# real-stanford/flingbot

Measured on AMD Instinct MI355X. Metric: sim steps/sec (64x64-particle cloth), higher is better.
Workload: dtype f32

## Files before the change

flingbot_amd/csrc/fs_fused_grid_kernel.h:

```cpp
#pragma once
#include "fs_fused_kernel.h"

#define FG_PLANE (FS_FUSED_MAX_PARTICLES * 4)
#define FG_PAD 1024
#define FG_OFF_XX FG_PAD
#define FG_OFF_X0 (FG_OFF_XX + 4 * FG_PLANE)
#define FG_OFF_CUR (FG_OFF_X0 + 3 * FG_PLANE)
#define FG_OFF_ITEMS (FG_OFF_CUR + FS_FUSED_CUR_BYTES)
#define FG_OFF_SCAN (FG_OFF_ITEMS + FS_FUSED_MAX_PARTICLES * 2)
#define FG_OFF_CSET (FG_OFF_SCAN + 64)
#define FG_OFF_CACC (FG_OFF_CSET + FS_FUSED_CSET_CAP * 2)
#define FG_OFF_CHIST (FG_OFF_CACC + FS_FUSED_CSET_CAP * 16)
#define FG_OFF_ROWL (FG_OFF_CHIST + 512)
#define FG_OFF_KZ (FG_OFF_ROWL + 1024)
#define FG_OFF_KS (FG_OFF_KZ + 1024)
#define FG_OFF_COLL (FG_OFF_KS + 1024)
#define FG_OFF_RCNT (FG_OFF_COLL + 512)
#define FG_LDS_BYTES (FG_OFF_RCNT + 512)
static_assert(FG_OFF_ROWL % 8 == 0 && (FG_OFF_KZ - FG_OFF_ROWL) % 8 == 0, "row tables are read as ds_read_b64 pairs");
static_assert((FG_OFF_COLL - FG_OFF_KS) % 256 == 0, "column tables share one address, rows as ds_read2st64_b32 offsets");
static_assert(FG_LDS_BYTES <= 160 * 1024, "grid-64 kernel: the LDS of one CU");
#ifndef FG_SINGLES
#define FG_SINGLES 1
#endif
#define FG_SINGLES_LANES (FS_FUSED_THREADS - 64)
#define FG_SINGLES_ROOM ((FS_FUSED_CUR_BYTES + FS_FUSED_MAX_PARTICLES * 2) / 16)
#define FG_SINGLES_CAP (FG_SINGLES_ROOM < 2 * FG_SINGLES_LANES ? FG_SINGLES_ROOM : 2 * FG_SINGLES_LANES)
#ifndef FG_PREFETCH_CAND
#define FG_PREFETCH_CAND 2
#endif

#define FG_ROW(w, k) (2 * (w) + 32 * ((k) >> 1) + ((k) & 1))

template <int DZ>
__device__ __forceinline__ void fg_load_slot(unsigned a, fs_f2 &x0, fs_f2 &x1, fs_f2 &x2) {
    asm volatile("ds_read2st64_b32 %0, %1 offset0:%2 offset1:%3" : "=v"(x0) : "v"(a), "n"(DZ + 2), "n"(DZ + 3) : "memory");
    asm volatile("ds_read2st64_b32 %0, %1 offset0:%2 offset1:%3" : "=v"(x1) : "v"(a), "n"(DZ + 2 + 64), "n"(DZ + 3 + 64) : "memory");
    asm volatile("ds_read2st64_b32 %0, %1 offset0:%2 offset1:%3" : "=v"(x2) : "v"(a), "n"(DZ + 2 + 128), "n"(DZ + 3 + 128) : "memory");
}
template <int OFF>
__device__ __forceinline__ fs_f2 fg_load_rows(unsigned a) {
    static_assert(OFF >= 0 && OFF < 65536 && OFF % 8 == 0, "ds_read_b64 offset");
    fs_f2 r;
    asm volatile("ds_read_b64 %0, %1 offset:%2" : "=v"(r) : "v"(a), "n"(OFF) : "memory");
    return r;
}
template <int R0, int R1>
__device__ __forceinline__ fs_f2 fg_load_cols(unsigned a) {
    static_assert(R0 >= 0 && R0 < 256 && R1 >= 0 && R1 < 256, "ds_read2st64_b32 offsets");
    fs_f2 r;
    asm volatile("ds_read2st64_b32 %0, %1 offset0:%2 offset1:%3" : "=v"(r) : "v"(a), "n"(R0), "n"(R1) : "memory");
    return r;
}
#define FG_WAIT(N, A0, A1, A2) asm volatile("s_waitcnt lgkmcnt(" #N ")" : "+v"(A0), "+v"(A1), "+v"(A2))

#define FG_MIN_L2 1.17549435e-38f
__device__ __forceinline__ float fg_scale(float xi0, float xi1, float xi2, float xj0, float xj1, float xj2, float L, float k,
                                          float &l2) {
    const float ex = xi0 - xj0, ey = xi1 - xj1, ez = xi2 - xj2;
    l2 = fs_dot3(ex, ey, ez, ex, ey, ez);
    const float inv = __builtin_amdgcn_rsqf(l2);
    const float len = l2 * inv;
    const float C = len - L;
    return k * (C * inv);
}
__device__ __forceinline__ void fg_accum(float &d0, float &d1, float &d2, float xi0, float xi1, float xi2, float xj0, float xj1,
                                         float xj2, float sc) {
    const float ex = xi0 - xj0, ey = xi1 - xj1, ez = xi2 - xj2;
    d0 = FS_FMA(-ex, sc, d0);
    d1 = FS_FMA(-ey, sc, d1);
    d2 = FS_FMA(-ez, sc, d2);
}
__device__ __forceinline__ float fg_from_left(float v) {
    return __int_as_float(__builtin_amdgcn_update_dpp(0, __float_as_int(v), 0x138, 0xf, 0xf, true));
}
__device__ __forceinline__ float fg_from_right(float v) {
    return __int_as_float(__builtin_amdgcn_update_dpp(0, __float_as_int(v), 0x130, 0xf, 0xf, true));
}

__device__ __forceinline__ void fg_apply(const FsAcc &a, float relax, const float *rcnt, float &x0, float &x1, float &x2) {
    if (a.cnt > 0) {
        const float sc = a.cnt < 128 ? rcnt[a.cnt] : relax / (float)a.cnt;
        x0 = FS_FMA(a.d0, sc, x0); x1 = FS_FMA(a.d1, sc, x1); x2 = FS_FMA(a.d2, sc, x2);
    }
}

__global__ __launch_bounds__(FS_FUSED_THREADS) void fs_k_fused_grid64(const FsEnvDev *__restrict__ envs,
                                                                      const FsShapesDev *__restrict__ shapes, const int *ids,
                                                                      int n_steps) {
    static_assert(FS_FUSED_THREADS == 1024 && FS_FUSED_PPT == 4, "grid-64 kernel: 16 waves x 4 rows");
    extern __shared__ __attribute__((aligned(16))) char smem[];
    float *Xx = (float *)(smem + FG_OFF_XX);
    float *Xy = Xx + FS_FUSED_MAX_PARTICLES, *Xz = Xy + FS_FUSED_MAX_PARTICLES, *Xw = Xz + FS_FUSED_MAX_PARTICLES;
    float *X0x = (float *)(smem + FG_OFF_X0);
    float *X0y = X0x + FS_FUSED_MAX_PARTICLES;
    float *X0z = X0y + FS_FUSED_MAX_PARTICLES;
    unsigned short *cursor = (unsigned short *)(smem + FG_OFF_CUR);
    unsigned short *items = (unsigned short *)(smem + FG_OFF_ITEMS);
    int *wave_tot = (int *)(smem + FG_OFF_SCAN);
    float *rowL = (float *)(smem + FG_OFF_ROWL);

#ifdef FS_BLOCK_CLOCKS
    const unsigned long long tc_start = __builtin_amdgcn_s_memtime(), tr_start = __builtin_amdgcn_s_memrealtime();
#endif
#ifdef FS_TIMING
    unsigned long long ts_acc[16] = {0, 0, 0, 0, 0, 0, 0, 0, 0, 0, 0, 0, 0, 0, 0, 0};
    unsigned long long ts_last = __builtin_amdgcn_s_memtime();
#endif
    const int e = ids[blockIdx.x];
    if (e < 0) return;
    const FsEnvDev &E = envs[e];
    const FsShapesDev &sh = shapes[e];
    const FsFusedConsts c = fs_fused_consts(E, sh);
    const int n = c.n;
    const unsigned un = (unsigned)n;
    const int t = threadIdx.x, lane = t & 63, w = t >> 6;
    const int dimz = n >> 6;

    FsVec4 *const g_pos = E.pos, *const g_vel = E.vel;
    const FsVec4 *const g_rest = E.rest;
    const fs_gci g_phase = (fs_gci)E.phase;
    const fs_gi g_nlist = (fs_gi)E.nlist, g_ncount = (fs_gi)E.ncount;
    const fs_gci g_ell_j = (fs_gci)E.ell_j;
    const fs_gcf g_ell_len = (fs_gcf)E.ell_len, g_ell_k = (fs_gcf)E.ell_k;
    const fs_gcf g_L = (fs_gcf)E.g64_L;
    const int max_deg = E.max_deg;
    const fs_gcu g_near = (fs_gcu)E.restnear_w;

    int find_mode = 0;
    {
        const int ph0 = g_phase[0];
        int differs = 0;
        for (int i = t; i < n; i += FS_FUSED_THREADS) differs |= (g_phase[i] != ph0);
        if (t == 0) wave_tot[0] = 0;
        __syncthreads();
        if (differs) atomicOr(&wave_tot[0], 1);
        __syncthreads();
        const int mixed = wave_tot[0];
        __syncthreads();
        if (!mixed) {
            if (!(ph0 & FS_PHASE_SELF_COLLIDE)) find_mode = 3;
            else if (!(ph0 & FS_PHASE_SELF_COLLIDE_FILTER)) find_mode = 2;
            else if (E.restnear_ok == 2 && FS_STENCIL_FILTER) find_mode = 4;
            else if (E.restnear_ok) find_mode = 1;
        }
    }
    for (int q = t; q < FG_OFF_X0 / 4; q += FS_FUSED_THREADS) ((float *)smem)[q] = 0.0f;
    __syncthreads();
    for (int i = t; i < n; i += FS_FUSED_THREADS) {
        const FsVec4 p = fs_ld4(g_pos, i);
        Xx[i] = p.x; Xy[i] = p.y; Xz[i] = p.z; Xw[i] = p.w;
        X0x[i] = p.x; X0y[i] = p.y; X0z[i] = p.z;
    }
    if (t < 256) {
        const int r = t & 63, s = 8 + (t >> 6);
        rowL[t] = r < dimz ? g_L[(unsigned)s * un + (unsigned)(r * 64 + 2)] : 0.0f;
    }
    constexpr int XS_DX[4] = {-1, -2, +1, +2};
    constexpr int SH_DX[4] = {+1, -1, -1, +1}, SH_DZ[4] = {-1, -1, +1, +1};
    constexpr int ZS_DZ[4] = {-1, -2, +1, +2};
    float *colL = (float *)(smem + FG_OFF_COLL);
    if (t < 128) {
        const int col = t & 63, q = t >> 6;
        const int dxq = q == 0 ? -1 : -2;
        colL[t] = (unsigned)(col + dxq) < 64u ? g_L[(unsigned)q * un + (unsigned)(2 * 64 + col)] : 0.0f;
    }
    float *rcnt = (float *)(smem + FG_OFF_RCNT);
    if (t < 128) rcnt[t] = t > 0 ? c.relax / (float)t : 0.0f;
    if (t < 256) {
        const int c64 = t & 63, q = t >> 6;
        const int sdx = (q == 0 || q == 3) ? +1 : -1, sslot = q < 2 ? 2 + q : 4 + q;
        const int zdz = q < 2 ? -1 - q : q - 1;
        ((float *)(smem + FG_OFF_KS))[t] = (unsigned)(c64 + sdx) < 64u ? E.g64_kh[sslot] : 0.0f;
        ((float *)(smem + FG_OFF_KZ))[t] = (c64 < dimz && (unsigned)(c64 + zdz) < (unsigned)dimz) ? E.g64_kh[8 + q] : 0.0f;
    }
    const float kh0 = E.g64_kh[0], kh1 = E.g64_kh[1];
    unsigned nvalid = 0u;
#pragma unroll
    for (int k = 0; k < FS_FUSED_PPT; ++k) {
        const int row = FG_ROW(w, k);
        int cnt = 0;
#pragma unroll
        for (int q = 0; q < 4; ++q) {
            cnt += ((unsigned)(lane + XS_DX[q]) < 64u) ? 1 : 0;
            cnt += ((unsigned)(lane + SH_DX[q]) < 64u && (unsigned)(row + SH_DZ[q]) < (unsigned)dimz) ? 1 : 0;
            cnt += ((unsigned)(row + ZS_DZ[q]) < (unsigned)dimz) ? 1 : 0;
        }
        nvalid |= (unsigned)cnt << (8 * k);
    }
    __syncthreads();
    unsigned fastmask = 0u;
    {
        constexpr int cdx[FS_G64_SLOTS] = FS_G64_DX_LIST, cdz[FS_G64_SLOTS] = FS_G64_DZ_LIST;
#pragma unroll
        for (int k = 0; k < FS_FUSED_PPT; ++k) {
            const int row = FG_ROW(w, k), i = row * 64 + lane;
            bool differs = false;
            if (i < n) {
                const float wi = Xw[i];
                differs = !(wi > 0.0f);
#pragma unroll
                for (int q = 0; q < FS_G64_SLOTS; ++q) {
                    const bool in = (unsigned)(lane + cdx[q]) < 64u && (unsigned)(row + cdz[q]) < (unsigned)dimz;
                    if (in) differs |= Xw[i + cdz[q] * 64 + cdx[q]] != wi;
                }
            }
            if (i < n && __builtin_amdgcn_ballot_w64(differs) == 0ull) fastmask |= 1u << k;
        }
        fastmask = (unsigned)__builtin_amdgcn_readfirstlane((int)fastmask);
    }

    FS_TS(0)
#pragma unroll 1
    for (int frame = 0; frame < n_steps; ++frame) {
#pragma unroll 1
        for (int sub = 0; sub < c.substeps; ++sub) {
            for (int q = t; q < FS_FUSED_BUCKETS / 2; q += FS_FUSED_THREADS) ((unsigned *)cursor)[q] = 0u;
            FsVec4 xp[FS_FUSED_PPT];
#pragma unroll
            for (int k = 0; k < FS_FUSED_PPT; ++k) {
                const int i = t + k * FS_FUSED_THREADS;
                xp[k] = FsVec4{0.0f, 0.0f, 0.0f, 0.0f};
                if (i < n) {
                    const FsVec4 p0 = FsVec4{X0x[i], X0y[i], X0z[i], Xw[i]};
                    xp[k] = fs_fused_predict(c, p0, fs_ld4(g_vel, i));
                    fs_st4(E.x0, i, p0);
                }
            }
            __syncthreads();
            fs_fused_build_grid(c, xp, cursor, items, wave_tot, X0x, X0y, X0z);
            FS_TS(1)
            const FsFindConsts fc = {n, c.ncap, c.rad2, c.inv_rad, find_mode, E.gp_dimx, E.gp_magic};
#pragma unroll 1
            for (int qs = t; qs < n; qs += FS_FUSED_THREADS) {
                const int i = items[qs];
                const FsVec4 xi = FsVec4{X0x[qs], X0y[qs], X0z[qs], 0.0f};
                const int shape_bits = (int)(fs_shape_candidates(E.p, sh, sub, xi.x, xi.y, xi.z) << FS_SHAPE_MASK_SHIFT);
                if (find_mode == 4) {
                    FsNearWords none;
#pragma unroll
                    for (int q = 0; q < 8; ++q) none.w[q] = 0xffffffffu;
                    g_ncount[i] = fs_fused_find_neighbors<true>(fc, i, xi, (fs_lcus)cursor, (fs_lcus)items, g_phase, g_rest, g_nlist,
                                                                none, (fs_lus)(smem + FG_OFF_XX) + t, (fs_lcf)X0x) | shape_bits;
                    continue;
                }
                FsNearWords near;
#pragma unroll
                for (int q = 0; q < 8; ++q) near.w[q] = find_mode == 1 ? g_near[(unsigned)q * un + (unsigned)i] : 0xffffffffu;
                g_ncount[i] = (find_mode == 3 ? 0
                                              : fs_fused_find_neighbors<false>(fc, i, xi, (fs_lcus)cursor, (fs_lcus)items, g_phase,
                                                                               g_rest, g_nlist, near,
                                                                               (fs_lus)(smem + FG_OFF_XX) + t, (fs_lcf)X0x)) |
                              shape_bits;
            }
            FS_TS(2)
            __syncthreads();
            FS_TS(3)
#pragma unroll
            for (int k = 0; k < FS_FUSED_PPT; ++k) {
                const int i = t + k * FS_FUSED_THREADS;
                if (i < n) {
                    Xx[i] = xp[k].x; Xy[i] = xp[k].y; Xz[i] = xp[k].z; Xw[i] = xp[k].w;
                    const FsVec4 p0 = fs_ld4(E.x0, i);
                    X0x[i] = p0.x; X0y[i] = p0.y; X0z[i] = p0.z;
                } else {
                    Xx[i] = 0.0f; Xy[i] = 0.0f; Xz[i] = 0.0f; Xw[i] = 0.0f;
                }
            }

            unsigned short *cset = (unsigned short *)(smem + FG_OFF_CSET);
            FsVec4 *cacc = (FsVec4 *)(smem + FG_OFF_CACC);
            int *chist = (int *)(smem + FG_OFF_CHIST);
            if (t < 128) chist[t] = 0;
            int *nsingles = (int *)(smem + FG_OFF_SCAN);
            if (t == 0) *nsingles = 0;
            __syncthreads();
            int ccls[FS_FUSED_PPT];
#pragma unroll
            for (int k = 0; k < FS_FUSED_PPT; ++k) {
                const int i = FG_ROW(w, k) * 64 + lane;
                int cc = 0;
                if (i < n && Xw[i] > 0.0f) cc = g_ncount[i] & FS_NCOUNT_MASK;
                ccls[k] = cc > 96 ? 96 : cc;
                if (ccls[k] > 0) atomicAdd(&chist[ccls[k]], 1);
            }
            __syncthreads();
            fs_fused_count_offsets(chist, t);
            __syncthreads();
            unsigned long long slotpack = ~0ull;
#pragma unroll
            for (int k = 0; k < FS_FUSED_PPT; ++k) {
                if (ccls[k] > 0) {
                    const int pos = atomicAdd(&chist[ccls[k]], 1);
                    if (pos < FS_FUSED_CSET_CAP) {
                        cset[pos] = (unsigned short)(FG_ROW(w, k) * 64 + lane);
                        slotpack = (slotpack & ~(0xffffull << (16 * k))) | ((unsigned long long)pos << (16 * k));
                    }
#if FG_SINGLES
                    else if (ccls[k] <= 16) {
                        const int sp = atomicAdd(nsingles, 1);
                        if (sp < FG_SINGLES_CAP)
                            slotpack = (slotpack & ~(0xffffull << (16 * k))) | ((unsigned long long)(FS_FUSED_CSET_CAP + sp) << (16 * k));
                    }
#endif
                }
            }
            __syncthreads();
            const int csize = chist[0] < FS_FUSED_CSET_CAP ? chist[0] : FS_FUSED_CSET_CAP;
            const int n_singles = *nsingles < FG_SINGLES_CAP ? *nsingles : FG_SINGLES_CAP;
            FsVec4 *squeue = (FsVec4 *)(smem + FG_OFF_CUR);
            const int i2 = t < csize ? (int)cset[t] : -1;
            int cnt2 = 0, cj2[FS_FUSED_PREFETCH_CAND];
            unsigned smask2 = 0u;
#pragma unroll
            for (int q = 0; q < FS_FUSED_PREFETCH_CAND; ++q) cj2[q] = 0;
            if (i2 >= 0) {
                const int word = g_ncount[i2];
                cnt2 = word & FS_NCOUNT_MASK;
                smask2 = (unsigned)word >> FS_SHAPE_MASK_SHIFT;
#pragma unroll
                for (int q = 0; q < FS_FUSED_PREFETCH_CAND; ++q) cj2[q] = g_nlist[(unsigned)q * un + (unsigned)i2];
            }

            FS_TS(4)
#pragma unroll 1
            for (int it = 0; it < c.iters; ++it) {
                int cntP, cntQ, cjP[FG_PREFETCH_CAND], cjQ[FG_PREFETCH_CAND];
                {
                    const int r0 = FG_ROW(w, 0) * 64 + lane;
                    unsigned i0 = r0 < n ? (unsigned)r0 : 0u, i1 = r0 + 64 < n ? (unsigned)(r0 + 64) : 0u;
                    asm volatile("" : "+v"(i0), "+v"(i1));
                    cntP = g_ncount[i0];
                    cntQ = g_ncount[i1];
#pragma unroll
                    for (int q = 0; q < FG_PREFETCH_CAND; ++q) {
                        cjP[q] = g_nlist[(unsigned)q * un + i0];
                        cjQ[q] = g_nlist[(unsigned)q * un + i1];
                    }
                }
                float rx[FS_FUSED_PPT], ry[FS_FUSED_PPT], rz[FS_FUSED_PPT];
#pragma unroll
                for (int q = 0; q < FS_FUSED_PPT; ++q) { rx[q] = 0.0f; ry[q] = 0.0f; rz[q] = 0.0f; }
#ifdef FG_UNROLL_PAIRS
#pragma unroll
#else
#pragma unroll 1
#endif
                for (int pr = 0; pr < 2; ++pr) {
                    const int rowP = FG_ROW(w, 2 * pr);
                    const int iP_raw = rowP * 64 + lane, iQ_raw = iP_raw + 64;
                    const bool haveP = rowP < dimz, haveQ = rowP + 1 < dimz;
                    const int iP = haveP ? iP_raw : 0, iQ = haveQ ? iQ_raw : 0;
                    const bool fast = haveQ && ((fastmask >> (2 * pr)) & 3u) == 3u;
                    const fs_f2 xi0 = fs_f2{Xx[iP], Xx[iQ]}, xi1 = fs_f2{Xy[iP], Xy[iQ]}, xi2 = fs_f2{Xz[iP], Xz[iQ]};
                    const fs_f2 wi = fs_f2{Xw[iP], Xw[iQ]};
                    FsAcc aP, aQ;
                    bool exact = !fast;
                    if (fast) {
                        unsigned aLane = (unsigned)(lane * 4);
                        asm volatile("" : "+v"(aLane));
                        const unsigned am2 = (unsigned)(FG_OFF_XX + ((rowP - 2) * 64 - 2) * 4) + aLane;
                        const unsigned am1 = am2 + 4u, a00 = am2 + 8u, ap1 = am2 + 12u, ap2 = am2 + 16u;
                        constexpr int SH_SLOT[4] = {2, 3, 6, 7};
                        float sLP[2], sLQ[4];
#pragma unroll
                        for (int q = 0; q < 2; ++q) sLP[q] = g_L[(unsigned)SH_SLOT[q] * un + (unsigned)iP];
#pragma unroll
                        for (int q = 0; q < 4; ++q) sLQ[q] = g_L[(unsigned)SH_SLOT[q] * un + (unsigned)iQ];
                        const unsigned aRow = (unsigned)(FG_OFF_ROWL + rowP * 4), aCol = (unsigned)FG_OFF_KS + aLane;
                        constexpr int CL_ROW = (FG_OFF_COLL - FG_OFF_KS) / 256;
                        fs_f2 cL = fg_load_cols<CL_ROW, CL_ROW + 1>(aCol);
                        const unsigned aKP = rowP >= 1 ? aCol : aLane;
                        const unsigned aKQ = rowP + 2 < dimz ? aCol : aLane;
                        fs_f2 kP23 = fg_load_cols<0, 1>(aKP);
                        fs_f2 kQ23 = fg_load_cols<0, 1>(aCol);
#define FG_KX(q) ((unsigned)(lane + XS_DX[q]) < 64u ? (q == 0 ? kh0 : kh1) : 0.0f)
                        float dP0 = 0.0f, dP1 = 0.0f, dP2 = 0.0f, dQ0 = 0.0f, dQ1 = 0.0f, dQ2 = 0.0f, mP = 1.0f, mQ = 1.0f;
                        fs_f2 u0, u1, u2, v0, v1, v2;
                        float l2a, l2b, l2c, l2d;
                        fg_load_slot<0>(am1, u0, u1, u2);
                        fg_load_slot<0>(am2, v0, v1, v2);
                        asm volatile("s_waitcnt lgkmcnt(3)"
                                     : "+v"(cL), "+v"(kP23), "+v"(kQ23), "+v"(u0), "+v"(u1), "+v"(u2));
                        const float scP0 = fg_scale(xi0.x, xi1.x, xi2.x, u0.x, u1.x, u2.x, cL.x, FG_KX(0), l2a);
                        const float scQ0 = fg_scale(xi0.y, xi1.y, xi2.y, u0.y, u1.y, u2.y, cL.x, FG_KX(0), l2b);
                        fg_accum(dP0, dP1, dP2, xi0.x, xi1.x, xi2.x, u0.x, u1.x, u2.x, scP0);
                        fg_accum(dQ0, dQ1, dQ2, xi0.y, xi1.y, xi2.y, u0.y, u1.y, u2.y, scQ0);
                        __builtin_amdgcn_sched_barrier(0);
                        fg_load_slot<-1>(ap1, u0, u1, u2);
                        FG_WAIT(3, v0, v1, v2);
                        const float scP1 = fg_scale(xi0.x, xi1.x, xi2.x, v0.x, v1.x, v2.x, cL.y, FG_KX(1), l2c);
                        const float scQ1 = fg_scale(xi0.y, xi1.y, xi2.y, v0.y, v1.y, v2.y, cL.y, FG_KX(1), l2d);
                        fg_accum(dP0, dP1, dP2, xi0.x, xi1.x, xi2.x, v0.x, v1.x, v2.x, scP1);
                        fg_accum(dQ0, dQ1, dQ2, xi0.y, xi1.y, xi2.y, v0.y, v1.y, v2.y, scQ1);
                        mP = fminf(fminf(mP, l2a), l2c);
                        mQ = fminf(fminf(mQ, l2b), l2d);
                        __builtin_amdgcn_sched_barrier(0);
                        fg_load_slot<-1>(am1, v0, v1, v2);
                        FG_WAIT(3, u0, u1, u2);
                        const float scQ2 = fg_scale(xi0.y, xi1.y, xi2.y, u0.y, u1.y, u2.y, sLQ[0], kQ23.x, l2b);
                        {
                            const float sc = fg_scale(xi0.x, xi1.x, xi2.x, u0.x, u1.x, u2.x, sLP[0], kP23.x, l2a);
                            fg_accum(dP0, dP1, dP2, xi0.x, xi1.x, xi2.x, u0.x, u1.x, u2.x, sc);
                        }
                        fg_accum(dQ0, dQ1, dQ2, xi0.y, xi1.y, xi2.y, u0.y, u1.y, u2.y, scQ2);
                        __builtin_amdgcn_sched_barrier(0);
                        fg_load_slot<0>(ap1, u0, u1, u2);
                        FG_WAIT(3, v0, v1, v2);
                        const float scQ3 = fg_scale(xi0.y, xi1.y, xi2.y, v0.y, v1.y, v2.y, sLQ[1], kQ23.y, l2d);
                        {
                            const float sc = fg_scale(xi0.x, xi1.x, xi2.x, v0.x, v1.x, v2.x, sLP[1], kP23.y, l2c);
                            fg_accum(dP0, dP1, dP2, xi0.x, xi1.x, xi2.x, v0.x, v1.x, v2.x, sc);
                        }
                        fg_accum(dQ0, dQ1, dQ2, xi0.y, xi1.y, xi2.y, v0.y, v1.y, v2.y, scQ3);
                        mP = fminf(fminf(mP, l2a), l2c);
                        mQ = fminf(fminf(mQ, l2b), l2d);
                        __builtin_amdgcn_sched_barrier(0);
                        fg_load_slot<0>(ap2, v0, v1, v2);
                        FG_WAIT(3, u0, u1, u2);
                        fg_accum(dP0, dP1, dP2, xi0.x, xi1.x, xi2.x, u0.x, u1.x, u2.x, fg_from_right(scP0));
                        fg_accum(dQ0, dQ1, dQ2, xi0.y, xi1.y, xi2.y, u0.y, u1.y, u2.y, fg_from_right(scQ0));
                        __builtin_amdgcn_sched_barrier(0);
                        fs_f2 kQ67 = fg_load_cols<2, 3>(aKQ);
                        fg_load_slot<+1>(am1, u0, u1, u2);
                        FG_WAIT(3, v0, v1, v2);
                        fg_accum(dP0, dP1, dP2, xi0.x, xi1.x, xi2.x, v0.x, v1.x, v2.x, fg_from_right(fg_from_right(scP1)));
                        fg_accum(dQ0, dQ1, dQ2, xi0.y, xi1.y, xi2.y, v0.y, v1.y, v2.y, fg_from_right(fg_from_right(scQ1)));
                        __builtin_amdgcn_sched_barrier(0);
                        fg_load_slot<+1>(ap1, v0, v1, v2);
                        asm volatile("s_waitcnt lgkmcnt(3)" : "+v"(kQ67), "+v"(u0), "+v"(u1), "+v"(u2));
                        fg_accum(dP0, dP1, dP2, xi0.x, xi1.x, xi2.x, u0.x, u1.x, u2.x, fg_from_left(scQ2));
                        {
                            const float sc = fg_scale(xi0.y, xi1.y, xi2.y, u0.y, u1.y, u2.y, sLQ[2], kQ67.x, l2a);
                            fg_accum(dQ0, dQ1, dQ2, xi0.y, xi1.y, xi2.y, u0.y, u1.y, u2.y, sc);
                        }
                        __builtin_amdgcn_sched_barrier(0);
                        constexpr int KZ = FG_OFF_KZ - FG_OFF_ROWL;
                        fs_f2 zL[4], zK[4];
                        zL[0] = fg_load_rows<0>(aRow); zK[0] = fg_load_rows<KZ>(aRow);
                        zL[1] = fg_load_rows<256>(aRow); zK[1] = fg_load_rows<KZ + 256>(aRow);
                        fg_load_slot<-1>(a00, u0, u1, u2);
                        asm volatile("s_waitcnt lgkmcnt(3)"
                                     : "+v"(zL[0]), "+v"(zK[0]), "+v"(zL[1]), "+v"(zK[1]), "+v"(v0), "+v"(v1), "+v"(v2));
                        fg_accum(dP0, dP1, dP2, xi0.x, xi1.x, xi2.x, v0.x, v1.x, v2.x, fg_from_right(scQ3));
                        {
                            const float sc = fg_scale(xi0.y, xi1.y, xi2.y, v0.y, v1.y, v2.y, sLQ[3], kQ67.y, l2b);
                            fg_accum(dQ0, dQ1, dQ2, xi0.y, xi1.y, xi2.y, v0.y, v1.y, v2.y, sc);
                        }
                        mQ = fminf(fminf(mQ, l2a), l2b);
                        __builtin_amdgcn_sched_barrier(0);
                        fg_load_slot<-2>(a00, v0, v1, v2);
                        FG_WAIT(3, u0, u1, u2);
                        const float scQ8 = fg_scale(xi0.y, xi1.y, xi2.y, u0.y, u1.y, u2.y, zL[0].y, zK[0].y, l2b);
                        {
                            const float sc = fg_scale(xi0.x, xi1.x, xi2.x, u0.x, u1.x, u2.x, zL[0].x, zK[0].x, l2a);
                            fg_accum(dP0, dP1, dP2, xi0.x, xi1.x, xi2.x, u0.x, u1.x, u2.x, sc);
                        }
                        fg_accum(dQ0, dQ1, dQ2, xi0.y, xi1.y, xi2.y, u0.y, u1.y, u2.y, scQ8);
                        __builtin_amdgcn_sched_barrier(0);
                        zL[2] = fg_load_rows<512>(aRow); zK[2] = fg_load_rows<KZ + 512>(aRow);
                        zL[3] = fg_load_rows<768>(aRow); zK[3] = fg_load_rows<KZ + 768>(aRow);
                        fg_load_slot<+1>(a00, u0, u1, u2);
                        asm volatile("s_waitcnt lgkmcnt(3)"
                                     : "+v"(zL[2]), "+v"(zK[2]), "+v"(zL[3]), "+v"(zK[3]), "+v"(v0), "+v"(v1), "+v"(v2));
                        {
                            const float sc = fg_scale(xi0.x, xi1.x, xi2.x, v0.x, v1.x, v2.x, zL[1].x, zK[1].x, l2c);
                            const float sd = fg_scale(xi0.y, xi1.y, xi2.y, v0.y, v1.y, v2.y, zL[1].y, zK[1].y, l2d);
                            fg_accum(dP0, dP1, dP2, xi0.x, xi1.x, xi2.x, v0.x, v1.x, v2.x, sc);
                            fg_accum(dQ0, dQ1, dQ2, xi0.y, xi1.y, xi2.y, v0.y, v1.y, v2.y, sd);
                        }
                        mP = fminf(fminf(mP, l2a), l2c);
                        mQ = fminf(fminf(mQ, l2b), l2d);
                        __builtin_amdgcn_sched_barrier(0);
                        fg_load_slot<+2>(a00, v0, v1, v2);
                        FG_WAIT(3, u0, u1, u2);
                        fg_accum(dP0, dP1, dP2, xi0.x, xi1.x, xi2.x, u0.x, u1.x, u2.x, scQ8);
                        {
                            const float sd = fg_scale(xi0.y, xi1.y, xi2.y, u0.y, u1.y, u2.y, zL[2].y, zK[2].y, l2c);
                            fg_accum(dQ0, dQ1, dQ2, xi0.y, xi1.y, xi2.y, u0.y, u1.y, u2.y, sd);
                        }
                        __builtin_amdgcn_sched_barrier(0);
                        FG_WAIT(0, v0, v1, v2);
                        {
                            const float sc = fg_scale(xi0.x, xi1.x, xi2.x, v0.x, v1.x, v2.x, zL[3].x, zK[3].x, l2a);
                            const float sd = fg_scale(xi0.y, xi1.y, xi2.y, v0.y, v1.y, v2.y, zL[3].y, zK[3].y, l2b);
                            fg_accum(dP0, dP1, dP2, xi0.x, xi1.x, xi2.x, v0.x, v1.x, v2.x, sc);
                            fg_accum(dQ0, dQ1, dQ2, xi0.y, xi1.y, xi2.y, v0.y, v1.y, v2.y, sd);
                        }
                        mP = fminf(mP, l2a);
                        mQ = fminf(fminf(mQ, l2c), l2b);
                        __builtin_amdgcn_sched_barrier(0);
#undef FG_KX
                        exact = __builtin_amdgcn_ballot_w64(mP < FG_MIN_L2 || mQ < FG_MIN_L2) != 0ull;
                        aP = FsAcc{dP0, dP1, dP2, (int)((nvalid >> (16 * pr)) & 0xffu)};
                        aQ = FsAcc{dQ0, dQ1, dQ2, (int)((nvalid >> (16 * pr + 8)) & 0xffu)};
                    }
                    if (exact) {
                        aP = FsAcc{0.0f, 0.0f, 0.0f, 0};
                        aQ = FsAcc{0.0f, 0.0f, 0.0f, 0};
                        if (haveP && wi.x > 0.0f)
                            for (int s = 0; s < max_deg; ++s) {
                                const int j = g_ell_j[(unsigned)s * un + (unsigned)iP];
                                if (j < 0) break;
                                fs_spring(aP, xi0.x, xi1.x, xi2.x, wi.x, FsVec4{Xx[j], Xy[j], Xz[j], Xw[j]},
                                          g_ell_len[(unsigned)s * un + (unsigned)iP], g_ell_k[(unsigned)s * un + (unsigned)iP]);
                            }
                        if (haveQ && wi.y > 0.0f)
                            for (int s = 0; s < max_deg; ++s) {
                                const int j = g_ell_j[(unsigned)s * un + (unsigned)iQ];
                                if (j < 0) break;
                                fs_spring(aQ, xi0.y, xi1.y, xi2.y, wi.y, FsVec4{Xx[j], Xy[j], Xz[j], Xw[j]},
                                          g_ell_len[(unsigned)s * un + (unsigned)iQ], g_ell_k[(unsigned)s * un + (unsigned)iQ]);
                            }
                    }
                    FS_TS(5)
                    int cntP_n, cntQ_n, cjP_n[FG_PREFETCH_CAND], cjQ_n[FG_PREFETCH_CAND];
                    {
                        const unsigned i0 = iP_raw + 2048 < n ? (unsigned)(iP_raw + 2048) : 0u;
                        const unsigned i1 = iQ_raw + 2048 < n ? (unsigned)(iQ_raw + 2048) : 0u;
                        cntP_n = g_ncount[i0];
                        cntQ_n = g_ncount[i1];
#pragma unroll
                        for (int q = 0; q < FG_PREFETCH_CAND; ++q) {
                            cjP_n[q] = g_nlist[(unsigned)q * un + i0];
                            cjQ_n[q] = g_nlist[(unsigned)q * un + i1];
                        }
                    }
                    FS_TS(12)
#pragma unroll
                    for (int h = 0; h < 2; ++h) {
                        const int i = h == 0 ? iP : iQ;
                        const bool have = h == 0 ? haveP : haveQ;
                        const float xi0s = h == 0 ? xi0.x : xi0.y, xi1s = h == 0 ? xi1.x : xi1.y, xi2s = h == 0 ? xi2.x : xi2.y;
                        const float wis = h == 0 ? wi.x : wi.y;
                        FsAcc a = h == 0 ? aP : aQ;
                        const int cntw = h == 0 ? cntP : cntQ;
                        const int cnt = cntw & FS_NCOUNT_MASK;
                        const unsigned smask = (unsigned)cntw >> FS_SHAPE_MASK_SHIFT;
                        int cj[FG_PREFETCH_CAND];
#pragma unroll
                        for (int q = 0; q < FG_PREFETCH_CAND; ++q) cj[q] = h == 0 ? cjP[q] : cjQ[q];
                        float nx = xi0s, ny = xi1s, nz = xi2s;
                        const unsigned myslot = (unsigned)(slotpack >> (16 * (2 * pr + h))) & 0xffffu;
                        if (wis > 0.0f && myslot < (unsigned)FS_FUSED_CSET_CAP && have) {
                            cacc[myslot] = FsVec4{a.d0, a.d1, a.d2, __int_as_float(a.cnt)};
                        } else if (wis > 0.0f && myslot != 0xffffu && have) {
                            squeue[myslot - FS_FUSED_CSET_CAP] =
                                FsVec4{a.d0, a.d1, a.d2, __int_as_float(i | (cj[0] << 12) | (a.cnt << 24) | ((cnt - 1) << 28))};
                        } else if (wis > 0.0f) {
                            const float ri0 = xi0s - X0x[i], ri1 = xi1s - X0y[i], ri2 = xi2s - X0z[i];
#pragma unroll 1
                            for (int q = 0; q < FG_PREFETCH_CAND && q < cnt; ++q) {
                                const int j = cj[0];
#pragma unroll
                                for (int r = 0; r + 1 < FG_PREFETCH_CAND; ++r) cj[r] = cj[r + 1];
                                const FsVec4 xj = FsVec4{Xx[j], Xy[j], Xz[j], Xw[j]};
                                fs_particle_contact(a, xi0s, xi1s, xi2s, wis, ri0, ri1, ri2, xj, xj.x - X0x[j], xj.y - X0y[j],
                                                    xj.z - X0z[j], c.restd, c.restd2, c.mu_p);
                            }
                            if (cnt > FG_PREFETCH_CAND) {
#pragma unroll 1
                                for (int sq = FG_PREFETCH_CAND; sq < cnt; ++sq) {
                                    const int j = g_nlist[(unsigned)sq * un + (unsigned)i];
                                    const FsVec4 xj = FsVec4{Xx[j], Xy[j], Xz[j], Xw[j]};
                                    fs_particle_contact(a, xi0s, xi1s, xi2s, wis, ri0, ri1, ri2, xj, xj.x - X0x[j],
                                                        xj.y - X0y[j], xj.z - X0z[j], c.restd, c.restd2, c.mu_p);
                                }
                            }
                            fs_fused_shape_contacts(a, c, E.p, sh, sub, smask, xi0s, xi1s, xi2s, ri0, ri1, ri2);
                            fg_apply(a, c.relax, rcnt, nx, ny, nz);
                        }
#pragma unroll
                        for (int q = FS_FUSED_PPT - 1; q > 0; --q) { rx[q] = rx[q - 1]; ry[q] = ry[q - 1]; rz[q] = rz[q - 1]; }
                        rx[0] = nx; ry[0] = ny; rz[0] = nz;
                        if (h == 0) { FS_TS(13) }
                    }
                    FS_TS(6)
                    cntP = cntP_n;
                    cntQ = cntQ_n;
#pragma unroll
                    for (int q = 0; q < FG_PREFETCH_CAND; ++q) { cjP[q] = cjP_n[q]; cjQ[q] = cjQ_n[q]; }
                }
                __syncthreads();
                FS_TS(7)
                float n2x = 0.0f, n2y = 0.0f, n2z = 0.0f;
                if (i2 >= 0) {
                    const float xi0 = Xx[i2], xi1 = Xy[i2], xi2 = Xz[i2], wi = Xw[i2];
                    const FsVec4 pa = cacc[t];
                    FsAcc a = {pa.x, pa.y, pa.z, __float_as_int(pa.w)};
                    const float ri0 = xi0 - X0x[i2], ri1 = xi1 - X0y[i2], ri2 = xi2 - X0z[i2];
                    int cjt[FS_FUSED_PREFETCH_CAND];
#pragma unroll
                    for (int q = 0; q < FS_FUSED_PREFETCH_CAND; ++q) cjt[q] = cj2[q];
                    for (int s0 = 0; s0 < cnt2; s0 += FS_FUSED_PREFETCH_CAND) {
                        int cn[FS_FUSED_PREFETCH_CAND];
#pragma unroll
                        for (int q = 0; q < FS_FUSED_PREFETCH_CAND; ++q) {
                            const int sn = s0 + FS_FUSED_PREFETCH_CAND + q;
                            cn[q] = sn < cnt2 ? g_nlist[(unsigned)sn * un + (unsigned)i2] : 0;
                        }
#pragma unroll 1
                        for (int q = 0; q < FS_FUSED_PREFETCH_CAND && s0 + q < cnt2; ++q) {
                            const int j = cjt[0];
#pragma unroll
                            for (int r = 0; r + 1 < FS_FUSED_PREFETCH_CAND; ++r) cjt[r] = cjt[r + 1];
                            const FsVec4 xj = FsVec4{Xx[j], Xy[j], Xz[j], Xw[j]};
                            fs_particle_contact(a, xi0, xi1, xi2, wi, ri0, ri1, ri2, xj, xj.x - X0x[j], xj.y - X0y[j],
                                                xj.z - X0z[j], c.restd, c.restd2, c.mu_p);
                        }
#pragma unroll
                        for (int q = 0; q < FS_FUSED_PREFETCH_CAND; ++q) cjt[q] = cn[q];
                    }
                    fs_fused_shape_contacts(a, c, E.p, sh, sub, smask2, xi0, xi1, xi2, ri0, ri1, ri2);
                    n2x = xi0; n2y = xi1; n2z = xi2;
                    fg_apply(a, c.relax, rcnt, n2x, n2y, n2z);
                }
#if FG_SINGLES
#pragma unroll 1
                for (int q = t - 64; q >= 0 && q < n_singles; q += FG_SINGLES_LANES) {
                    const FsVec4 pa = squeue[q];
                    const unsigned word = (unsigned)__float_as_int(pa.w);
                    const int i = (int)(word & 0xfffu), more = (int)(word >> 28);
                    int j = (int)((word >> 12) & 0xfffu);
                    int jn = more > 0 ? g_nlist[un + (unsigned)i] : 0;
                    const unsigned smask = (unsigned)g_ncount[i] >> FS_SHAPE_MASK_SHIFT;
                    FsAcc a = {pa.x, pa.y, pa.z, (int)((word >> 24) & 15u)};
                    float xi0 = Xx[i], xi1 = Xy[i], xi2 = Xz[i];
                    const float wi = Xw[i];
                    const float ri0 = xi0 - X0x[i], ri1 = xi1 - X0y[i], ri2 = xi2 - X0z[i];
#pragma unroll 1
                    for (int sq = 0; sq <= more; ++sq) {
                        const FsVec4 xj = FsVec4{Xx[j], Xy[j], Xz[j], Xw[j]};
                        fs_particle_contact(a, xi0, xi1, xi2, wi, ri0, ri1, ri2, xj, xj.x - X0x[j], xj.y - X0y[j], xj.z - X0z[j], c.restd,
                                            c.restd2, c.mu_p);
                        j = jn;
                        if (sq + 2 <= more) jn = g_nlist[(unsigned)(sq + 2) * un + (unsigned)i];
                    }
                    fs_fused_shape_contacts(a, c, E.p, sh, sub, smask, xi0, xi1, xi2, ri0, ri1, ri2);
                    fg_apply(a, c.relax, rcnt, xi0, xi1, xi2);
                    squeue[q] = FsVec4{xi0, xi1, xi2, pa.w};
                }
#endif
                FS_TS(8)
                __syncthreads();
                FS_TS(9)
#pragma unroll
                for (int q = 0; q < FS_FUSED_PPT; ++q) {
                    const int i = FG_ROW(w, q) * 64 + lane;
                    const bool in_set = ((unsigned)(slotpack >> (16 * q)) & 0xffffu) != 0xffffu;
                    if (i < n && !in_set) { Xx[i] = rx[FS_FUSED_PPT - 1 - q]; Xy[i] = ry[FS_FUSED_PPT - 1 - q]; Xz[i] = rz[FS_FUSED_PPT - 1 - q]; }
                }
                if (i2 >= 0) { Xx[i2] = n2x; Xy[i2] = n2y; Xz[i2] = n2z; }
#if FG_SINGLES
#pragma unroll 1
                for (int q = t - 64; q >= 0 && q < n_singles; q += FG_SINGLES_LANES) {
                    const FsVec4 pn = squeue[q];
                    const int i = __float_as_int(pn.w) & 0xfff;
                    Xx[i] = pn.x; Xy[i] = pn.y; Xz[i] = pn.z;
                }
#endif
                __syncthreads();
                FS_TS(10)
            }
            for (int i = t; i < n; i += FS_FUSED_THREADS) {
                const FsVec4 xf = FsVec4{Xx[i], Xy[i], Xz[i], Xw[i]};
                FsVec4 p0 = FsVec4{X0x[i], X0y[i], X0z[i], xf.w};
                FsVec4 v = fs_ld4(g_vel, i);
                fs_fused_finalize(c, p0, v, xf);
                fs_st4(g_vel, i, v);
                X0x[i] = p0.x; X0y[i] = p0.y; X0z[i] = p0.z;
            }
        }
    }
    for (int i = t; i < n; i += FS_FUSED_THREADS) fs_st4(g_pos, i, FsVec4{X0x[i], X0y[i], X0z[i], Xw[i]});
#ifdef FS_BLOCK_CLOCKS
    if (t == 0) {
        const unsigned long long tc_total = __builtin_amdgcn_s_memtime() - tc_start, tr_end = __builtin_amdgcn_s_memrealtime();
        const fs_gi out = g_nlist + 95u * un;
        out[0] = (int)(unsigned)tc_total; out[1] = (int)(unsigned)(tc_total >> 32);
        out[2] = (int)(unsigned)tr_start; out[3] = (int)(unsigned)tr_end;
    }
#endif
#ifdef FS_TIMING
    FS_TS(11)
    if (blockIdx.x == 0 && (t & 63) == 0)
        printf("TS wave %2d: init %llu grid %llu find %llu findwait %llu cset %llu springs %llu rest %llu bar1 %llu pass2 %llu bar2 %llu publish %llu final %llu | exact+prefetch %llu tailP %llu tailQ %llu\n",
               t >> 6, ts_acc[0], ts_acc[1], ts_acc[2], ts_acc[3], ts_acc[4], ts_acc[5], ts_acc[6] + ts_acc[12] + ts_acc[13], ts_acc[7], ts_acc[8],
               ts_acc[9], ts_acc[10], ts_acc[11], ts_acc[12], ts_acc[13], ts_acc[6]);
#endif
}
```

Baseline: 127,500.

## Split contact solve: park accumulators, then apply shape contacts in separate finish pass

The contact iteration is restructured so the spring phase now only parks partial accumulators (in registers, the cset accumulator array, or the singles queue). Shape contacts and the position update for every particle move into a unified finish pass after the second barrier. Inline-contact particles walk their full neighbour list directly instead of prefetching candidates for the next row pair. Singles queue words are precomputed once before the iteration loop. This cuts per-iteration global prefetch traffic and register pressure and balances the shape-contact work across all waves. In exchange it adds a third pass over the particles with extra LDS reads and more serial work after the barrier.

```diff
diff --git a/flingbot_amd/csrc/fs_fused_grid_kernel.h b/flingbot_amd/csrc/fs_fused_grid_kernel.h
--- a/flingbot_amd/csrc/fs_fused_grid_kernel.h
+++ b/flingbot_amd/csrc/fs_fused_grid_kernel.h
@@ -5,12 +5,12 @@
 #define FG_PAD 1024
 #define FG_OFF_XX FG_PAD
 #define FG_OFF_X0 (FG_OFF_XX + 4 * FG_PLANE)
-#define FG_OFF_CUR (FG_OFF_X0 + 3 * FG_PLANE)
+#define FG_OFF_CACC (FG_OFF_X0 + 3 * FG_PLANE)
+#define FG_OFF_CUR (FG_OFF_CACC + FS_FUSED_CSET_CAP * 16)
 #define FG_OFF_ITEMS (FG_OFF_CUR + FS_FUSED_CUR_BYTES)
 #define FG_OFF_SCAN (FG_OFF_ITEMS + FS_FUSED_MAX_PARTICLES * 2)
 #define FG_OFF_CSET (FG_OFF_SCAN + 64)
-#define FG_OFF_CACC (FG_OFF_CSET + FS_FUSED_CSET_CAP * 2)
-#define FG_OFF_CHIST (FG_OFF_CACC + FS_FUSED_CSET_CAP * 16)
+#define FG_OFF_CHIST (FG_OFF_CSET + FS_FUSED_CSET_CAP * 2)
 #define FG_OFF_ROWL (FG_OFF_CHIST + 512)
 #define FG_OFF_KZ (FG_OFF_ROWL + 1024)
 #define FG_OFF_KS (FG_OFF_KZ + 1024)
@@ -20,15 +20,16 @@
 static_assert(FG_OFF_ROWL % 8 == 0 && (FG_OFF_KZ - FG_OFF_ROWL) % 8 == 0, "row tables are read as ds_read_b64 pairs");
 static_assert((FG_OFF_COLL - FG_OFF_KS) % 256 == 0, "column tables share one address, rows as ds_read2st64_b32 offsets");
 static_assert(FG_LDS_BYTES <= 160 * 1024, "grid-64 kernel: the LDS of one CU");
+static_assert(FG_OFF_CACC % 16 == 0 && FG_OFF_CUR == FG_OFF_CACC + FS_FUSED_CSET_CAP * 16, "set and queue accumulators: one array");
 #ifndef FG_SINGLES
 #define FG_SINGLES 1
 #endif
 #define FG_SINGLES_LANES (FS_FUSED_THREADS - 64)
 #define FG_SINGLES_ROOM ((FS_FUSED_CUR_BYTES + FS_FUSED_MAX_PARTICLES * 2) / 16)
 #define FG_SINGLES_CAP (FG_SINGLES_ROOM < 2 * FG_SINGLES_LANES ? FG_SINGLES_ROOM : 2 * FG_SINGLES_LANES)
-#ifndef FG_PREFETCH_CAND
-#define FG_PREFETCH_CAND 2
-#endif
+#define FG_SLOT_NONE 0xffffu
+#define FG_SLOT_INLINE 0xfffeu
+static_assert(FS_FUSED_CSET_CAP + FG_SINGLES_CAP <= FG_SLOT_INLINE, "slot values below the reserved ones");
 
 #define FG_ROW(w, k) (2 * (w) + 32 * ((k) >> 1) + ((k) & 1))
 
@@ -287,57 +288,54 @@
             __syncthreads();
             fs_fused_count_offsets(chist, t);
             __syncthreads();
+            FsVec4 *squeue = cacc + FS_FUSED_CSET_CAP;
             unsigned long long slotpack = ~0ull;
 #pragma unroll
             for (int k = 0; k < FS_FUSED_PPT; ++k) {
                 if (ccls[k] > 0) {
+                    const int i = FG_ROW(w, k) * 64 + lane;
+                    unsigned slot = FG_SLOT_INLINE;
                     const int pos = atomicAdd(&chist[ccls[k]], 1);
                     if (pos < FS_FUSED_CSET_CAP) {
-                        cset[pos] = (unsigned short)(FG_ROW(w, k) * 64 + lane);
-                        slotpack = (slotpack & ~(0xffffull << (16 * k))) | ((unsigned long long)pos << (16 * k));
+                        cset[pos] = (unsigned short)i;
+                        slot = (unsigned)pos;
                     }
 #if FG_SINGLES
                     else if (ccls[k] <= 16) {
                         const int sp = atomicAdd(nsingles, 1);
-                        if (sp < FG_SINGLES_CAP)
-                            slotpack = (slotpack & ~(0xffffull << (16 * k))) | ((unsigned long long)(FS_FUSED_CSET_CAP + sp) << (16 * k));
-                    }
-#endif
+                        if (sp < FG_SINGLES_CAP) {
+                            slot = (unsigned)(FS_FUSED_CSET_CAP + sp);
+                            squeue[sp].w = __int_as_float(i | (g_nlist[i] << 12) | ((ccls[k] - 1) << 28));
+                        }
+                    }
+#endif
+                    slotpack = (slotpack & ~(0xffffull << (16 * k))) | ((unsigned long long)slot << (16 * k));
                 }
             }
             __syncthreads();
             const int csize = chist[0] < FS_FUSED_CSET_CAP ? chist[0] : FS_FUSED_CSET_CAP;
             const int n_singles = *nsingles < FG_SINGLES_CAP ? *nsingles : FG_SINGLES_CAP;
-            FsVec4 *squeue = (FsVec4 *)(smem + FG_OFF_CUR);
             const int i2 = t < csize ? (int)cset[t] : -1;
             int cnt2 = 0, cj2[FS_FUSED_PREFETCH_CAND];
-            unsigned smask2 = 0u;
 #pragma unroll
             for (int q = 0; q < FS_FUSED_PREFETCH_CAND; ++q) cj2[q] = 0;
             if (i2 >= 0) {
-                const int word = g_ncount[i2];
-                cnt2 = word & FS_NCOUNT_MASK;
-                smask2 = (unsigned)word >> FS_SHAPE_MASK_SHIFT;
+                cnt2 = g_ncount[i2] & FS_NCOUNT_MASK;
 #pragma unroll
                 for (int q = 0; q < FS_FUSED_PREFETCH_CAND; ++q) cj2[q] = g_nlist[(unsigned)q * un + (unsigned)i2];
             }
+            static_assert(FG_SINGLES_CAP <= 2 * FG_SINGLES_LANES, "two queue entries per lane");
+            unsigned qw0 = 0u, qw1 = 0u;
+#if FG_SINGLES
+            if (t >= 64 && t - 64 < n_singles) qw0 = (unsigned)__float_as_int(squeue[t - 64].w);
+            if (t >= 64 && t - 64 + FG_SINGLES_LANES < n_singles) qw1 = (unsigned)__float_as_int(squeue[t - 64 + FG_SINGLES_LANES].w);
+            __syncthreads();
+#endif
 
             FS_TS(4)
 #pragma unroll 1
             for (int it = 0; it < c.iters; ++it) {
-                int cntP, cntQ, cjP[FG_PREFETCH_CAND], cjQ[FG_PREFETCH_CAND];
-                {
-                    const int r0 = FG_ROW(w, 0) * 64 + lane;
-                    unsigned i0 = r0 < n ? (unsigned)r0 : 0u, i1 = r0 + 64 < n ? (unsigned)(r0 + 64) : 0u;
-                    asm volatile("" : "+v"(i0), "+v"(i1));
-                    cntP = g_ncount[i0];
-                    cntQ = g_ncount[i1];
-#pragma unroll
-                    for (int q = 0; q < FG_PREFETCH_CAND; ++q) {
-                        cjP[q] = g_nlist[(unsigned)q * un + i0];
-                        cjQ[q] = g_nlist[(unsigned)q * un + i1];
-                    }
-                }
+                unsigned cpack = 0u;
                 float rx[FS_FUSED_PPT], ry[FS_FUSED_PPT], rz[FS_FUSED_PPT];
 #pragma unroll
                 for (int q = 0; q < FS_FUSED_PPT; ++q) { rx[q] = 0.0f; ry[q] = 0.0f; rz[q] = 0.0f; }
@@ -514,76 +512,43 @@
                             }
                     }
                     FS_TS(5)
-                    int cntP_n, cntQ_n, cjP_n[FG_PREFETCH_CAND], cjQ_n[FG_PREFETCH_CAND];
-                    {
-                        const unsigned i0 = iP_raw + 2048 < n ? (unsigned)(iP_raw + 2048) : 0u;
-                        const unsigned i1 = iQ_raw + 2048 < n ? (unsigned)(iQ_raw + 2048) : 0u;
-                        cntP_n = g_ncount[i0];
-                        cntQ_n = g_ncount[i1];
-#pragma unroll
-                        for (int q = 0; q < FG_PREFETCH_CAND; ++q) {
-                            cjP_n[q] = g_nlist[(unsigned)q * un + i0];
-                            cjQ_n[q] = g_nlist[(unsigned)q * un + i1];
-                        }
-                    }
-                    FS_TS(12)
 #pragma unroll
                     for (int h = 0; h < 2; ++h) {
                         const int i = h == 0 ? iP : iQ;
-                        const bool have = h == 0 ? haveP : haveQ;
-                        const float xi0s = h == 0 ? xi0.x : xi0.y, xi1s = h == 0 ? xi1.x : xi1.y, xi2s = h == 0 ? xi2.x : xi2.y;
-                        const float wis = h == 0 ? wi.x : wi.y;
                         FsAcc a = h == 0 ? aP : aQ;
-                        const int cntw = h == 0 ? cntP : cntQ;
-                        const int cnt = cntw & FS_NCOUNT_MASK;
-                        const unsigned smask = (unsigned)cntw >> FS_SHAPE_MASK_SHIFT;
-                        int cj[FG_PREFETCH_CAND];
-#pragma unroll
-                        for (int q = 0; q < FG_PREFETCH_CAND; ++q) cj[q] = h == 0 ? cjP[q] : cjQ[q];
-                        float nx = xi0s, ny = xi1s, nz = xi2s;
                         const unsigned myslot = (unsigned)(slotpack >> (16 * (2 * pr + h))) & 0xffffu;
-                        if (wis > 0.0f && myslot < (unsigned)FS_FUSED_CSET_CAP && have) {
+                        if (myslot < FG_SLOT_INLINE) {
                             cacc[myslot] = FsVec4{a.d0, a.d1, a.d2, __int_as_float(a.cnt)};
-                        } else if (wis > 0.0f && myslot != 0xffffu && have) {
-                            squeue[myslot - FS_FUSED_CSET_CAP] =
-                                FsVec4{a.d0, a.d1, a.d2, __int_as_float(i | (cj[0] << 12) | (a.cnt << 24) | ((cnt - 1) << 28))};
-                        } else if (wis > 0.0f) {
+                        } else if (myslot == FG_SLOT_INLINE) {
+                            const float xi0s = h == 0 ? xi0.x : xi0.y, xi1s = h == 0 ? xi1.x : xi1.y, xi2s = h == 0 ? xi2.x : xi2.y;
+                            const float wis = h == 0 ? wi.x : wi.y;
                             const float ri0 = xi0s - X0x[i], ri1 = xi1s - X0y[i], ri2 = xi2s - X0z[i];
-#pragma unroll 1
-                            for (int q = 0; q < FG_PREFETCH_CAND && q < cnt; ++q) {
-                                const int j = cj[0];
-#pragma unroll
-                                for (int r = 0; r + 1 < FG_PREFETCH_CAND; ++r) cj[r] = cj[r + 1];
+                            const int cnt = g_ncount[i] & FS_NCOUNT_MASK;
+#pragma unroll 1
+                            for (int sq = 0; sq < cnt; ++sq) {
+                                const int j = g_nlist[(unsigned)sq * un + (unsigned)i];
                                 const FsVec4 xj = FsVec4{Xx[j], Xy[j], Xz[j], Xw[j]};
                                 fs_particle_contact(a, xi0s, xi1s, xi2s, wis, ri0, ri1, ri2, xj, xj.x - X0x[j], xj.y - X0y[j],
                                                     xj.z - X0z[j], c.restd, c.restd2, c.mu_p);
                             }
-                            if (cnt > FG_PREFETCH_CAND) {
-#pragma unroll 1
-                                for (int sq = FG_PREFETCH_CAND; sq < cnt; ++sq) {
-                                    const int j = g_nlist[(unsigned)sq * un + (unsigned)i];
-                                    const FsVec4 xj = FsVec4{Xx[j], Xy[j], Xz[j], Xw[j]};
-                                    fs_particle_contact(a, xi0s, xi1s, xi2s, wis, ri0, ri1, ri2, xj, xj.x - X0x[j],
-                                                        xj.y - X0y[j], xj.z - X0z[j], c.restd, c.restd2, c.mu_p);
-                                }
-                            }
-                            fs_fused_shape_contacts(a, c, E.p, sh, sub, smask, xi0s, xi1s, xi2s, ri0, ri1, ri2);
-                            fg_apply(a, c.relax, rcnt, nx, ny, nz);
                         }
 #pragma unroll
                         for (int q = FS_FUSED_PPT - 1; q > 0; --q) { rx[q] = rx[q - 1]; ry[q] = ry[q - 1]; rz[q] = rz[q - 1]; }
-                        rx[0] = nx; ry[0] = ny; rz[0] = nz;
-                        if (h == 0) { FS_TS(13) }
+                        rx[0] = a.d0; ry[0] = a.d1; rz[0] = a.d2;
+                        cpack = (cpack << 8) | (unsigned)a.cnt;
                     }
                     FS_TS(6)
-                    cntP = cntP_n;
-                    cntQ = cntQ_n;
-#pragma unroll
-                    for (int q = 0; q < FG_PREFETCH_CAND; ++q) { cjP[q] = cjP_n[q]; cjQ[q] = cjQ_n[q]; }
                 }
                 __syncthreads();
                 FS_TS(7)
-                float n2x = 0.0f, n2y = 0.0f, n2z = 0.0f;
+                unsigned smk[FS_FUSED_PPT];
+#pragma unroll
+                for (int k = 0; k < FS_FUSED_PPT; ++k) {
+                    const int i = FG_ROW(w, k) * 64 + lane;
+                    unsigned ic = i < n ? (unsigned)i : 0u;
+                    asm volatile("" : "+v"(ic));
+                    smk[k] = (unsigned)g_ncount[ic] >> FS_SHAPE_MASK_SHIFT;
+                }
                 if (i2 >= 0) {
                     const float xi0 = Xx[i2], xi1 = Xy[i2], xi2 = Xz[i2], wi = Xw[i2];
                     const FsVec4 pa = cacc[t];
@@ -611,22 +576,18 @@
 #pragma unroll
                         for (int q = 0; q < FS_FUSED_PREFETCH_CAND; ++q) cjt[q] = cn[q];
                     }
-                    fs_fused_shape_contacts(a, c, E.p, sh, sub, smask2, xi0, xi1, xi2, ri0, ri1, ri2);
-                    n2x = xi0; n2y = xi1; n2z = xi2;
-                    fg_apply(a, c.relax, rcnt, n2x, n2y, n2z);
+                    cacc[t] = FsVec4{a.d0, a.d1, a.d2, __int_as_float(a.cnt)};
                 }
 #if FG_SINGLES
 #pragma unroll 1
-                for (int q = t - 64; q >= 0 && q < n_singles; q += FG_SINGLES_LANES) {
-                    const FsVec4 pa = squeue[q];
-                    const unsigned word = (unsigned)__float_as_int(pa.w);
+                for (int r = 0, q = t - 64; q >= 0 && q < n_singles; ++r, q += FG_SINGLES_LANES) {
+                    const unsigned word = r == 0 ? qw0 : qw1;
                     const int i = (int)(word & 0xfffu), more = (int)(word >> 28);
                     int j = (int)((word >> 12) & 0xfffu);
                     int jn = more > 0 ? g_nlist[un + (unsigned)i] : 0;
-                    const unsigned smask = (unsigned)g_ncount[i] >> FS_SHAPE_MASK_SHIFT;
-                    FsAcc a = {pa.x, pa.y, pa.z, (int)((word >> 24) & 15u)};
-                    float xi0 = Xx[i], xi1 = Xy[i], xi2 = Xz[i];
-                    const float wi = Xw[i];
+                    const FsVec4 pa = squeue[q];
+                    FsAcc a = {pa.x, pa.y, pa.z, __float_as_int(pa.w)};
+                    const float xi0 = Xx[i], xi1 = Xy[i], xi2 = Xz[i], wi = Xw[i];
                     const float ri0 = xi0 - X0x[i], ri1 = xi1 - X0y[i], ri2 = xi2 - X0z[i];
 #pragma unroll 1
                     for (int sq = 0; sq <= more; ++sq) {
@@ -636,29 +597,38 @@
                         j = jn;
                         if (sq + 2 <= more) jn = g_nlist[(unsigned)(sq + 2) * un + (unsigned)i];
                     }
-                    fs_fused_shape_contacts(a, c, E.p, sh, sub, smask, xi0, xi1, xi2, ri0, ri1, ri2);
-                    fg_apply(a, c.relax, rcnt, xi0, xi1, xi2);
-                    squeue[q] = FsVec4{xi0, xi1, xi2, pa.w};
+                    squeue[q] = FsVec4{a.d0, a.d1, a.d2, __int_as_float(a.cnt)};
                 }
 #endif
                 FS_TS(8)
                 __syncthreads();
                 FS_TS(9)
-#pragma unroll
-                for (int q = 0; q < FS_FUSED_PPT; ++q) {
-                    const int i = FG_ROW(w, q) * 64 + lane;
-                    const bool in_set = ((unsigned)(slotpack >> (16 * q)) & 0xffffu) != 0xffffu;
-                    if (i < n && !in_set) { Xx[i] = rx[FS_FUSED_PPT - 1 - q]; Xy[i] = ry[FS_FUSED_PPT - 1 - q]; Xz[i] = rz[FS_FUSED_PPT - 1 - q]; }
-                }
-                if (i2 >= 0) { Xx[i2] = n2x; Xy[i2] = n2y; Xz[i2] = n2z; }
-#if FG_SINGLES
-#pragma unroll 1
-                for (int q = t - 64; q >= 0 && q < n_singles; q += FG_SINGLES_LANES) {
-                    const FsVec4 pn = squeue[q];
-                    const int i = __float_as_int(pn.w) & 0xfff;
-                    Xx[i] = pn.x; Xy[i] = pn.y; Xz[i] = pn.z;
-                }
-#endif
+#pragma unroll 1
+                for (int k = 0; k < FS_FUSED_PPT; ++k) {
+                    const int i = FG_ROW(w, k) * 64 + lane;
+                    const unsigned myslot = (unsigned)(slotpack >> (16 * k)) & 0xffffu;
+                    FsAcc a = {rx[FS_FUSED_PPT - 1], ry[FS_FUSED_PPT - 1], rz[FS_FUSED_PPT - 1], (int)(cpack >> 8 * (FS_FUSED_PPT - 1))};
+                    const unsigned smask = smk[0];
+#pragma unroll
+                    for (int q = FS_FUSED_PPT - 1; q > 0; --q) { rx[q] = rx[q - 1]; ry[q] = ry[q - 1]; rz[q] = rz[q - 1]; }
+#pragma unroll
+                    for (int q = 0; q + 1 < FS_FUSED_PPT; ++q) smk[q] = smk[q + 1];
+                    cpack <<= 8;
+                    if (i < n) {
+                        const float wi = Xw[i];
+                        if (wi > 0.0f) {
+                            if (myslot < FG_SLOT_INLINE) {
+                                const FsVec4 pa = cacc[myslot];
+                                a = FsAcc{pa.x, pa.y, pa.z, __float_as_int(pa.w)};
+                            }
+                            float xi0 = Xx[i], xi1 = Xy[i], xi2 = Xz[i];
+                            const float ri0 = xi0 - X0x[i], ri1 = xi1 - X0y[i], ri2 = xi2 - X0z[i];
+                            fs_fused_shape_contacts(a, c, E.p, sh, sub, smask, xi0, xi1, xi2, ri0, ri1, ri2);
+                            fg_apply(a, c.relax, rcnt, xi0, xi1, xi2);
+                            Xx[i] = xi0; Xy[i] = xi1; Xz[i] = xi2;
+                        }
+                    }
+                }
                 __syncthreads();
                 FS_TS(10)
             }
@@ -684,8 +654,8 @@
 #ifdef FS_TIMING
     FS_TS(11)
     if (blockIdx.x == 0 && (t & 63) == 0)
-        printf("TS wave %2d: init %llu grid %llu find %llu findwait %llu cset %llu springs %llu rest %llu bar1 %llu pass2 %llu bar2 %llu publish %llu final %llu | exact+prefetch %llu tailP %llu tailQ %llu\n",
-               t >> 6, ts_acc[0], ts_acc[1], ts_acc[2], ts_acc[3], ts_acc[4], ts_acc[5], ts_acc[6] + ts_acc[12] + ts_acc[13], ts_acc[7], ts_acc[8],
-               ts_acc[9], ts_acc[10], ts_acc[11], ts_acc[12], ts_acc[13], ts_acc[6]);
-#endif
-}
+        printf("TS wave %2d: init %llu grid %llu find %llu findwait %llu cset %llu springs %llu park %llu bar1 %llu contact %llu bar2 %llu finish+bar3 %llu final %llu\n",
+               t >> 6, ts_acc[0], ts_acc[1], ts_acc[2], ts_acc[3], ts_acc[4], ts_acc[5], ts_acc[6], ts_acc[7], ts_acc[8], ts_acc[9], ts_acc[10],
+               ts_acc[11]);
+#endif
+}
```

Measured after the change: 132,000, median of 6. +3.5%, better.
